# kwea123/nerf_pl

Measured on AMD Instinct MI355X. Metric: rays/sec (64+128 samples), full training step: render_rays fwd + MSE + bwd + grad all-reduce + Adam, higher is better.
Workload: dtype bf16

## Files before the change

### nerf_pl_amd/csrc/mlp_render.hip

```cpp
#include "common.h"
#include "mlp_layout.h"

namespace nerfhip {
using namespace mlp;
typedef nerfhip_render_args RenderArgs;
constexpr int kRenderRays = 4;

template <int PREC, int SV>
int launch_render_variant(const RenderArgs& a, unsigned groups, hipStream_t stream);
template <> int launch_render_variant<NERFHIP_F32, 0>(const RenderArgs&, unsigned, hipStream_t);
template <> int launch_render_variant<NERFHIP_F32, 1>(const RenderArgs&, unsigned, hipStream_t);
template <> int launch_render_variant<NERFHIP_BF16, 0>(const RenderArgs&, unsigned, hipStream_t);
template <> int launch_render_variant<NERFHIP_BF16, 1>(const RenderArgs&, unsigned, hipStream_t);
template <> int launch_render_variant<NERFHIP_BF16, 2>(const RenderArgs&, unsigned, hipStream_t);
template <> int launch_render_variant<NERFHIP_F32, 3>(const RenderArgs&, unsigned, hipStream_t);
template <> int launch_render_variant<NERFHIP_BF16, 3>(const RenderArgs&, unsigned, hipStream_t);

static int render_tail_floats_host(int S_c, int N_i) {
    const int S_f = S_c + N_i;
    const int S4 = (S_c + 3) & ~3, N4 = (N_i + 3) & ~3, F4 = (S_f + 3) & ~3;
    const int fz = N_i > 0 ? 3 * S4 + N4 + ((S_c + 1 + 3) & ~3) + N4 : 0;
    const int coarse = 2 * S4 + fz;
    return coarse > F4 ? coarse : F4;
}

static bool render_shape_ok(int64_t B, int S_c, int N_i, int dtype) {
    if (dtype != NERFHIP_F32 && dtype != NERFHIP_BF16 && dtype != NERFHIP_BF16_F8) return false;
    const int pts = 32 * (dtype == NERFHIP_F32 ? 4 : 8);
    if (B <= 0 || B % kRenderRays != 0 || B / kRenderRays > 0x7fffffff || S_c < 3 || N_i < 0) return false;
    if ((kRenderRays * S_c) % pts != 0 || (N_i > 0 && (kRenderRays * (S_c + N_i)) % pts != 0)) return false;
    if ((int64_t)B * (S_c + N_i) / pts > 0x7fffffff) return false;
    return (size_t)kRenderRays * render_tail_floats_host(S_c, N_i) * sizeof(float) <= (size_t)kSlots * kChunkBytes;
}

static int render_check(const RenderArgs* a, int dtype, bool train) {
    NERFHIP_CHECK_ARG(a != nullptr);
    if (!render_shape_ok(a->B, a->S_c, a->N_i, dtype)) return NERFHIP_E_UNSUPPORTED;
    const bool fine = a->N_i > 0;
    NERFHIP_CHECK_ARG(a->rays && a->packed_coarse && a->z_coarse && a->raw_coarse && a->opacity_coarse);
    NERFHIP_CHECK_ARG(!fine || (a->packed_fine && a->z_fine && a->raw_fine && a->rgb_fine && a->depth_fine && a->opacity_fine));
    NERFHIP_CHECK_ARG(a->perturb <= 0.0f || a->perturb_rand);
    NERFHIP_CHECK_ARG(a->noise_std == 0.0f || (a->noise_coarse && (!fine || a->noise_fine)));
    NERFHIP_CHECK_ARG(a->row_total == NERFHIP_ROW_TOTAL_EXACT || a->row_total == NERFHIP_ROW_TOTAL_ATEN);
    if (train)
        NERFHIP_CHECK_ARG(a->target && a->rgb_coarse && a->depth_coarse && a->g_raw_coarse && a->save_coarse && a->out3 && a->ticket &&
                          (!fine || (a->g_raw_fine && a->save_fine)));
    uintptr_t lines = (uintptr_t)a->z_coarse | (uintptr_t)a->raw_coarse | (uintptr_t)a->z_fine | (uintptr_t)a->raw_fine;
    if (train) lines |= (uintptr_t)a->g_raw_coarse | (uintptr_t)a->g_raw_fine;
    if ((lines & 127) || (((uintptr_t)a->packed_coarse | (uintptr_t)a->packed_fine) & 15)) return NERFHIP_E_ALIGN;
    return 0;
}

}

extern "C" int nerfhip_render_supported(int64_t B, int S_c, int N_i, int dtype) {
    return nerfhip::render_shape_ok(B, S_c, N_i, dtype) ? 1 : 0;
// ... 34 lines not shown
```

### nerf_pl_amd/csrc/mlp_render_kernel.h

```cpp
#pragma once
#include "composite_wave.h"
#include "mlp_fwd_kernel.h"

namespace nerfhip {

constexpr int kRenderRays = 4;

typedef nerfhip_render_args RenderArgs;

__host__ __device__ inline int render_tail_floats(int S_c, int N_i, int S_f) {
    const int S4 = (S_c + 3) & ~3, N4 = (N_i + 3) & ~3, F4 = (S_f + 3) & ~3;
    const int fz = N_i > 0 ? 3 * S4 + N4 + ((S_c + 1 + 3) & ~3) + N4 : 0;
    const int coarse = 2 * S4 + fz;
    return coarse > F4 ? coarse : F4;
}

__device__ __forceinline__ void render_wg_sync() {
    asm volatile("s_waitcnt vmcnt(0) lgkmcnt(0)\n\ts_barrier" ::: "memory");
}

typedef const RenderArgs __attribute__((address_space(4)))* RenderArgsP;
__device__ __forceinline__ RenderArgsP render_args() {
    RenderArgsP p = (RenderArgsP)__builtin_amdgcn_kernarg_segment_ptr();
    asm volatile("" : "+s"(p));
    return p;
}

template <bool TRAIN, int NW, bool TT = false>
__device__ __forceinline__ void render_tail(const bool fine_pass, const bool with_fine_z, float* const tail_lds, const int wave,
                                            const int lane) {
    constexpr int R = kRenderRays;
    const RenderArgsP a = render_args();
    const int S_c = a->S_c, N_i = a->N_i, S_f = S_c + N_i;
    const float noise_std = a->noise_std;
    const float* raw = fine_pass ? a->raw_fine : a->raw_coarse;
    const float* z = fine_pass ? a->z_fine : a->z_coarse;
    const float* noise = noise_std != 0.0f ? (fine_pass ? a->noise_fine : a->noise_coarse) : nullptr;
    const int S = fine_pass ? S_f : S_c;
    float* rgb = fine_pass ? a->rgb_fine : a->rgb_coarse;
    float* depth = fine_pass ? a->depth_fine : a->depth_coarse;
    float* opac = fine_pass ? a->opacity_fine : a->opacity_coarse;
    const float* rays = a->rays;
    const int white_back = a->white_back;
    const int per_ray = render_tail_floats(S_c, N_i, S_f);
    const int S4 = (S_c + 3) & ~3;
    const int64_t ray0 = (int64_t)blockIdx.x * R, B = a->B;
    const int njobs = with_fine_z ? 2 * R : R;
    for (int job = wave; job < njobs; job += NW) {
        const int slot = job < R ? job : job - R;
        const int64_t r = ray0 + slot;
        if (r >= B) continue;
        float* base = tail_lds + (size_t)slot * per_ray;
        if (job < R) {
            if constexpr (TRAIN) {
                composite_train_wave<true>(raw, z, rays, noise, noise_std, white_back, a->target, a->grad_scale, nullptr, rgb, depth, opac,
                                           fine_pass ? a->g_raw_fine : a->g_raw_coarse, r, S, base, nullptr, lane);
            } else if (TT && !fine_pass) {
                composite_fwd_wave<1>(raw, z, rays, noise, noise_std, white_back, nullptr, nullptr, nullptr, opac, r, S, nullptr, lane);
            } else {
                composite_fwd_wave<4>(raw, z, rays, noise, noise_std, white_back, nullptr, rgb, depth, opac, r, S, nullptr, lane);
            }
        } else {
            float* w_s = base + S4;
            composite_weights_wave<(TT ? 1 : 4)>(raw, z, rays, noise, noise_std, r, S, w_s, lane);
            __builtin_amdgcn_wave_barrier();
            const float* u = a->u;
            fine_z_wave(w_s + S4, z + r * S, [&](int j) { return w_s[1 + j]; }, u ? u + r * a->u_stride : nullptr, S, N_i, a->eps,
                        a->z_fine + r * S_f, nullptr, nullptr, nullptr, lane, a->row_total);
        }
    }
}

template <int PREC, int SV>
__global__ __launch_bounds__(PrecTraits<PREC>::NW * 64, PrecTraits<PREC>::WPS)
void mlp_render_kernel(const RenderArgs args_by_value) {
    constexpr bool TRAIN = SV == 1 || SV == 2, TT = SV == 3;
    constexpr int FSV = TT ? 0 : SV;
    constexpr int NW = PrecTraits<PREC>::NW, PTS = 32 * NW, R = kRenderRays;
    __shared__ __attribute__((aligned(1024))) char lds_all[FwdLds<PREC, TRAIN>::kBytes];
    __shared__ float red[2][16];
    __shared__ unsigned last_s;
    const int lane = threadIdx.x & 63;
    const int wave = __builtin_amdgcn_readfirstlane((int)(threadIdx.x >> 6));
    float* const tail_lds = reinterpret_cast<float*>(lds_all + FwdLds<PREC, TRAIN>::kRingOff);
    int nc, nf;
    {
        const RenderArgsP a = render_args();
        const int S_c = a->S_c, N_i = a->N_i;
        nc = R * S_c / PTS;
        nf = N_i > 0 ? R * (S_c + N_i) / PTS : 0;
    }
    const int total = nc + nf;
#pragma clang loop unroll(disable)
    for (int sp = 0; sp < total; ++sp) {
        if (sp > 0) render_wg_sync();
        if (sp == nc) {
            render_tail<TRAIN, NW, TT>(false, true, tail_lds, wave, lane);
            render_wg_sync();
        }
        const RenderArgsP a = render_args();
        const bool fine = sp >= nc;
        const int S = fine ? a->S_c + a->N_i : a->S_c;
        const unsigned blk = fine ? blockIdx.x * (unsigned)nf + (unsigned)(sp - nc) : blockIdx.x * (unsigned)nc + (unsigned)sp;
        const FwdZGen zg{fine ? nullptr : a->perturb_rand, fine ? nullptr : a->z_coarse, fine ? 0 : a->use_disp, fine ? 0.0f : a->perturb,
                          TRAIN ? a->regen_enc : 0};
        uint8_t* save = nullptr;
        if constexpr (TRAIN) save = (uint8_t*)(fine ? a->save_fine : a->save_coarse);
        if (TT && !fine)
            mlp_fwd_body<PREC, MODE_RAYS, true, 0>(lds_all, blk, a->rays, nullptr, a->B * (int64_t)S, (int64_t)S, (const uint8_t*)a->packed_coarse,
                                                   a->raw_coarse, nullptr, zg);
        else
            mlp_fwd_body<PREC, MODE_RAYS, false, FSV>(lds_all, blk, a->rays, fine ? a->z_fine : nullptr, a->B * (int64_t)S, (int64_t)S,
                                                      (const uint8_t*)(fine ? a->packed_fine : a->packed_coarse), fine ? a->raw_fine : a->raw_coarse, save, zg);
    }
    render_wg_sync();
    render_tail<TRAIN, NW, TT>(nf > 0, false, tail_lds, wave, lane);

    if constexpr (TRAIN) {
        const RenderArgsP a = render_args();
        unsigned* const ticket = a->ticket;
        asm volatile("s_waitcnt vmcnt(0)" ::: "memory");
        __syncthreads();
        if (threadIdx.x == 0) {
            const unsigned prev = __hip_atomic_fetch_add(ticket, 1u, __ATOMIC_RELAXED, __HIP_MEMORY_SCOPE_AGENT);
            last_s = (prev == gridDim.x - 1) ? 1u : 0u;
            if (prev == gridDim.x - 1) __hip_atomic_store(ticket, 0u, __ATOMIC_RELAXED, __HIP_MEMORY_SCOPE_AGENT);
        }
        __syncthreads();
        if (!last_s) return;
        __builtin_amdgcn_fence(__ATOMIC_ACQUIRE, "agent");
        const float* img_c = a->rgb_coarse;
        const float* img_f = a->rgb_fine;
        const float* target = a->target;
        float* out3 = a->out3;
        const int64_t n3 = 3 * a->B;
        auto fresh_c = [&](int64_t i) { return __hip_atomic_load(img_c + i, __ATOMIC_RELAXED, __HIP_MEMORY_SCOPE_AGENT); };
        auto fresh_f = [&](int64_t i) { return __hip_atomic_load(img_f + i, __ATOMIC_RELAXED, __HIP_MEMORY_SCOPE_AGENT); };
        constexpr int Q = 1024 / (NW * 64);
        if (nf > 0)
            mse_psnr_block<Q>(fresh_c, fresh_f, true, target, n3, out3, nullptr, nullptr, red);
        else
            mse_psnr_block<Q>(fresh_c, [&](int64_t i) { return 0.0f; }, false, target, n3, out3, nullptr, nullptr, red);
    }
}

template <int PREC, int SV>
int launch_render_variant(const RenderArgs& a, unsigned groups, hipStream_t stream);

}
// ... 1 lines not shown
```

### nerf_pl_amd/csrc/sampling_wave.h

```cpp
#pragma once
#include "sampling_math.h"

namespace nerfhip {

template <typename P>
__device__ __forceinline__ int lower_bound(P a, int n, float v) {
    int lo = 0, hi = n;
    while (lo < hi) {
        const int mid = (lo + hi) >> 1;
        if (a[mid] < v) lo = mid + 1; else hi = mid;
    }
    return lo;
}
template <typename P>
__device__ __forceinline__ int upper_bound(P a, int n, float v) {
    int lo = 0, hi = n;
    while (lo < hi) {
        const int mid = (lo + hi) >> 1;
        if (a[mid] <= v) lo = mid + 1; else hi = mid;
    }
    return lo;
}

constexpr int ROW_TOTAL_EXACT = 0, ROW_TOTAL_ATEN = 1;
// ... 61 lines not shown
        for (int j = lane; j < M; j += 64) part += (double)nh_add(wload(j), eps);
        total = (float)wave_sum(part);
    }
    double carry = 0.0;
    for (int j0 = 0; j0 < M; j0 += 64) {
        const int j = j0 + lane;
        const float pdf = (j < M) ? nh_div(nh_add(wload(j), eps), total) : 0.0f;
        const double incl = wave_incl_sum((double)pdf, lane) + carry;
        if (j < M) cdf_s[j + 1] = (float)incl;
        carry = __shfl(incl, 63, 64);
    }
    if (lane == 0) cdf_s[0] = 0.0f;
    __builtin_amdgcn_wave_barrier();
}

__device__ __forceinline__ float invert_cdf(const float* cdf_s, const float* bins_s, int M, float u, float eps,
                                            int* ind_out = nullptr) {
    const int ind = upper_bound(cdf_s, M + 1, u);
    if (ind_out) *ind_out = ind;
    const int below = max(ind - 1, 0);
    const int above = min(ind, M);
    const float cb = cdf_s[below], ca = cdf_s[above];
    const float bb = bins_s[below], ba = bins_s[above];
    float denom = nh_sub(ca, cb);
    if (denom < eps) denom = 1.0f;
    const float t = nh_div(nh_sub(u, cb), denom);
    return nh_add(bb, nh_mul(t, nh_sub(ba, bb)));
}

__device__ __forceinline__ int fine_z_lds_floats(int S, int N) {
    const int S4 = (S + 3) & ~3, N4 = (N + 3) & ~3;
    return 3 * S4 + N4 + ((S + 1 + 3) & ~3) + N4;
}
template <typename WLoad>
__device__ __forceinline__ void fine_z_wave(float* lds, const float* __restrict__ zrow, WLoad wload, const float* __restrict__ urow,
                                            int S, int N, float eps, float* __restrict__ out, float* __restrict__ znew,
                                            float* __restrict__ cdf_row, int64_t* __restrict__ inds_row, int lane,
                                            int row_total = ROW_TOTAL_EXACT) {
    const int M = S - 2;
    const int S4 = (S + 3) & ~3, N4 = (N + 3) & ~3, H4 = (S + 1 + 3) & ~3;
    float* zc_s = lds;
    float* cdf_s = zc_s + S4;
    float* bins_s = cdf_s + S4;
    float* zn_s = bins_s + S4;
    int* hist_s = reinterpret_cast<int*>(zn_s + N4);
    int* ub_s = hist_s + H4;
    for (int j = lane; j < S; j += 64) zc_s[j] = zrow[j];
    for (int j = lane; j <= S; j += 64) hist_s[j] = 0;
    if (lane < N4 - N) zn_s[N + lane] = __builtin_inff();
    __builtin_amdgcn_wave_barrier();
    for (int j = lane; j < S - 1; j += 64) bins_s[j] = nh_mul(0.5f, nh_add(zc_s[j], zc_s[j + 1]));
    build_cdf_wave(wload, M, eps, cdf_s, lane, row_total);
    if (cdf_row)
        for (int j = lane; j <= M; j += 64) cdf_row[j] = cdf_s[j];
    for (int k = lane; k < N; k += 64) {
        const float uk = urow ? urow[k] : linspace01(k, N);
        int ind;
        const float v = invert_cdf(cdf_s, bins_s, M, uk, eps, &ind);
        if (inds_row) inds_row[k] = (int64_t)ind;
        zn_s[k] = v;
        if (znew) znew[k] = v;
        const int ub = upper_bound(zc_s, S, v);
        ub_s[k] = ub;
        atomicAdd(&hist_s[ub], 1);
    }
    __builtin_amdgcn_wave_barrier();
    int carry = 0;
    for (int i0 = 0; i0 < S; i0 += 64) {
        const int i = i0 + lane;
        int c = (i < S) ? hist_s[i] : 0;
#pragma unroll
        for (int o = 1; o < 64; o <<= 1) {
            const int t = __shfl_up(c, o, 64);
            if (lane >= o) c += t;
        }
        c += carry;
        if (i < S) out[i + c] = zc_s[i];
        carry = __shfl(c, 63, 64);
    }
    bool in_order = true;
    for (int k = lane; k < N; k += 64) in_order = in_order && (k == 0 || zn_s[k - 1] <= zn_s[k]);
    if (__all(in_order)) {
        for (int k = lane; k < N; k += 64) out[ub_s[k] + k] = zn_s[k];
        return;
    }
    const float4* zn4 = reinterpret_cast<const float4*>(zn_s);
    for (int k = lane; k < N; k += 64) {
        const float x = zn_s[k];
        int rank = ub_s[k];
#pragma unroll 4
        for (int q4 = 0; q4 < N4 / 4; ++q4) {
            const float4 y = zn4[q4];
            const int q = q4 * 4;
            rank += (y.x < x || (y.x == x && q + 0 < k)) ? 1 : 0;
            rank += (y.y < x || (y.y == x && q + 1 < k)) ? 1 : 0;
            rank += (y.z < x || (y.z == x && q + 2 < k)) ? 1 : 0;
            rank += (y.w < x || (y.w == x && q + 3 < k)) ? 1 : 0;
        }
        out[rank] = x;
    }
}

}
```

### nerf_pl_amd/csrc/mlp_bwd_chain.hip

```cpp
#include "mlp_device.h"
#include "f8_store.h"
#include "mlp_bwd_chain.h"

namespace nerfhip {

__device__ __forceinline__ float slab_absmax8(const bf16x8& s) {
    float m = 0.0f;
#pragma unroll
    for (int j = 0; j < 8; ++j) m = fmaxf(m, fabsf((float)s[j]));
    return m;
}
__device__ __forceinline__ float slab_absmax8(const f32x8& s) { return 0.0f; }

constexpr int kChainDepthBf16 = 2, kChainDepthF8 = 0;
constexpr int kChainBurst = 2;
template <int PREC> using BwdStream = RingStream<PrecTraits<PREC>::NW, bwd_chunks(PREC), true>;

template <typename Slab>
__device__ __forceinline__ Slab load_slab(__amdgpu_buffer_rsrc_t rsrc, int sec, int lane) {
    Slab s;
    u32x4* dst = reinterpret_cast<u32x4*>(&s);
    const unsigned voff = (unsigned)lane * (unsigned)sizeof(Slab);
    const unsigned soff = (unsigned)(sec * 64 * sizeof(Slab));
#pragma unroll
// ... 203 lines not shown
    st.wave = wave;
    st.pending = 0;
    st.pending_prev = 0;
    st.issue_chunk(0);
    st.issue_chunk(1);
    const unsigned lds_lo = (unsigned)(uintptr_t)ring + (unsigned)lane * 16u;
    unsigned lds_hi = lds_lo + 65536u;
    asm volatile("" : "+v"(lds_hi));
    const unsigned sig_lds = (unsigned)(uintptr_t)ring + (unsigned)(kSlots * kChunkBytes) + (unsigned)((wave * 64 + lane) * (int)sizeof(Slab));

    float v[8];
    Slab zero_slab;
#pragma unroll
    for (int j = 0; j < 8; ++j) v[j] = 0.0f;
    make_slab(zero_slab, v);
    Slab g_rgb, g_sig;
    {
        const float ga[3] = {g.x * o.x * (1.0f - o.x), g.y * o.y * (1.0f - o.y), g.z * o.z * (1.0f - o.z)};
#pragma unroll
        for (int j = 0; j < 8; ++j) v[j] = (h == 0 && j < 3) ? ga[j < 3 ? j : 0] : 0.0f;
        make_slab(g_rgb, v);
#pragma unroll
        for (int j = 0; j < 8; ++j) v[j] = (h == 0 && j == 0) ? g.w : 0.0f;
        make_slab(g_sig, v);
    }
    if constexpr (F8) {
        if constexpr (PREC == NERFHIP_BF16) {
            const int sb_rgb = bf8_block_scale(slab_absmax8(g_rgb)), sb_sig = bf8_block_scale(slab_absmax8(g_sig));
            save_pair_bf8(st.pending, dy_tile, kDyRgb / 2, g_rgb, zero_slab, sb_rgb, lane);
            save_pair_bf8(st.pending, dy_tile, kDySigma / 2, g_sig, zero_slab, sb_sig, lane);
            save_scale_f8(st.pending, dy_tile, f8_dy_scale_off(), f8_dy_section(kDyRgb), sb_rgb, lane);
            save_scale_f8(st.pending, dy_tile, f8_dy_scale_off(), f8_dy_section(kDySigma), sb_sig, lane);
        }
    } else {
        store_slab<PREC>(st.pending, dys, kDyRgb, g_rgb, lane);
        store_slab<PREC>(st.pending, dys, kDyRgb + 1, zero_slab, lane);
        store_slab<PREC>(st.pending, dys, kDySigma, g_sig, lane);
        store_slab<PREC>(st.pending, dys, kDySigma + 1, zero_slab, lane);
    }

    Slab gd[8];
    Slab ga[16], gb[16];
    Slab g_in0[1] = {g_rgb};
    int sb = run_bwd_layer_tm<PREC, 0, 4, 1, true, F8, 0>(st, lds_lo, lds_hi, sig_lds, g_in0, gd, acts, kGateOff, kMaskPieceT, dys, dy_tile, kDyDir,
                                                          f8_dy_section(kDyDir), -1, 127, lane);
    *reinterpret_cast<__attribute__((address_space(3))) Slab*>(sig_lds) = g_sig;
    static_assert(kBwdLayerFold == 1, "layer sequence below");
    sb = run_bwd_layer_tm<PREC, 1, 8, 9, true, F8, 4>(st, lds_lo, lds_hi, sig_lds, gd, gb, acts, kGateOff, mask_piece_h(8), dys, dy_tile, dy_h(8),
                                                      f8_dy_section(dy_h(8)), kDyDir, sb, lane);
    static_assert(bwd_layer_pieces(2, PREC) * 3 % (kChunkPieces * kSlots) == 0, "three looped layers = a whole number of ring turns");
#define NH_BWD(L, IN, OUT, D)                                                                                                \
    sb = run_bwd_layer_tm<PREC, L, 8, 16, true, F8, 8>(st, lds_lo, lds_hi, sig_lds, reinterpret_cast<const Slab(&)[16]>(IN), OUT, acts, kGateOff, \
                                                       mask_piece_h(9 - L) - (D), dys, dy_tile, dy_h(9 - L) + 16 * (D),              \
                                                       f8_dy_section(dy_h(9 - L)) + (D), dy_h(10 - L) + 16 * (D), sb, lane);
    if constexpr (PREC != NERFHIP_BF16) {
        NH_BWD(2, gb, ga, 0) NH_BWD(3, ga, gb, 0) NH_BWD(4, gb, ga, 0) NH_BWD(5, ga, gb, 0) NH_BWD(6, gb, ga, 0) NH_BWD(7, ga, gb, 0)
    } else {
        const uint8_t* const gsrc0 = st.gsrc;
        int n_pass;
        asm volatile("s_mov_b32 %0, 2" : "=s"(n_pass));
#pragma clang loop unroll(disable)
        for (int pass = 0; pass < n_pass; ++pass) {
            st.pending = 0;
            st.pending_prev = 0;
            const int d = 3 * pass;
            NH_BWD(2, gb, ga, d) NH_BWD(3, ga, gb, d) NH_BWD(4, gb, ga, d)
// ... 49 lines not shown
```

### nerf_pl_amd/csrc/mlp_bwd_dw.hip

```cpp
#include "mlp_device.h"
#include "mlp_bwd_dw.h"

namespace nerfhip {

#if NERFHIP_DW_PROBE
__device__ unsigned g_dw_probe[1024 * 8 * 8];
#endif

constexpr int kDwRingKiB = 160, kDwMaxDepth = 12;
constexpr int kDwFragRing = 5, kDwFragRing2D = 4;

template <int PREC> struct DwTraits;
template <> struct DwTraits<NERFHIP_BF16> {
    static constexpr int SPP = 1;
    static constexpr int RING_BYTES = kDwRingKiB * 1024;
    static constexpr int DEPTH = 0, STAGE_BYTES = 0;
};
template <> struct DwTraits<NERFHIP_F32> {
    static constexpr int SPP = 2;
    static constexpr int DEPTH = 2;
    static constexpr int MAXP = 72;
    static constexpr int STAGE_BYTES = MAXP * kPieceBytes;
    static constexpr int RING_BYTES = DEPTH * STAGE_BYTES;
};
// ... 76 lines not shown
    const int64_t my_tiles = (t_first >= ntiles) ? 0 : ((ntiles - t_first < per) ? ntiles - t_first : per);
    const unsigned lds_base = (unsigned)(uintptr_t)ring;

    const int dma_off_even = (PREC == NERFHIP_BF16) ? ((lane & 1) * 32 + (lane >> 1)) * 16 : lane * 16;
    const int dma_off_odd = (PREC == NERFHIP_BF16) ? ((lane & 1) * 32 + ((lane ^ 8) >> 1)) * 16 : lane * 16;

    f32x16 acc[kDwMaxXTiles];
#pragma unroll
    for (int x = 0; x < kDwMaxXTiles; ++x)
#pragma unroll
        for (int r = 0; r < 16; ++r) acc[x][r] = 0.0f;
    float dbacc = 0.0f;
    [[maybe_unused]] float dbacc2 = 0.0f;

    const int grp = lane >> 4, c = lane & 15;
    const int tr_off = (grp & 1) * SLAB_BYTES + (2 * (8 * (grp >> 1) + (c >> 2)) + ((c & 3) & 1)) * 16 + ((c & 3) >> 1) * 8;
    const int tr_s0 = (grp & 1) ? 128 : 0, tr_s1 = 128 - tr_s0;
    [[maybe_unused]] auto load_frag = [&](const char* pb, int q) { return load_frag_tr16(pb, tr_off, tr_s0, tr_s1, q); };
    const int m32 = lane & 31, kk = lane >> 5;
    const int f32_off = (m32 >> 4) * SLAB_BYTES + (slab_nat_h(m32 & 15) * 32) * 32 + slab_nat_j(m32 & 15) * 4;
#if NERFHIP_DW_PROBE
    unsigned pr_wait = 0, pr_bar = 0, pr_issue = 0, pr_comp = 0, pr_depth = 0;
    const uint64_t pr_t00 = __builtin_amdgcn_s_memrealtime();
#endif

    auto run = [&](auto nxt_c, auto nsl_c, auto regen_c) {
        constexpr int NXT = decltype(nxt_c)::value, NSL = decltype(nsl_c)::value;
        constexpr bool REGEN = decltype(regen_c)::value;
        static_assert(!REGEN || (PREC == NERFHIP_BF16 && (NXT == 2 || NXT == 9 || NXT == 10)), "classes with an encoding section");
        constexpr int ENC = REGEN ? (NXT == 9 ? kDirSlabs : kXyzSlabs) : 0;
        constexpr int DYS = NXT == 9 ? 8 : 16;
        constexpr bool FOLD = NXT == 9 && NSL == kDwFoldStageSlabs;
        constexpr bool SPLIT2D = (PREC == NERFHIP_BF16) && (NXT == 8 || NXT == 10) && (NSL - 2 * NXT >= 16);
        constexpr int NP = NSL * SPP;
        constexpr int NPD = NP - ENC;
        constexpr int LPWD = (NPD + 7) / 8;
        constexpr int LPW = LPWD + (REGEN ? 1 : 0);
        constexpr int STAGE = (PREC == NERFHIP_BF16) ? NP * kPieceBytes : DwTraits<PREC>::STAGE_BYTES;
        constexpr int ZSLOT = 256;
        constexpr int D0 = dw_depth<PREC>(NP);
        constexpr int D = (REGEN && D0 * (STAGE + ZSLOT) > RING_BYTES) ? D0 - 1 : D0;
        static_assert(D >= 2 && D * (STAGE + (REGEN ? ZSLOT : 0)) <= RING_BYTES, "ring stages of this job class");
        static_assert((D - 2) * LPW <= 63, "counted vmcnt");
#if NERFHIP_DW_PROBE
        pr_depth = D;
#endif
        int s_issue = 0, s_use = 0;
        const uint8_t* abase = nullptr;
        const uint8_t* dbase = nullptr;
        unsigned slot = 0;
        auto stage_tile = [&](int64_t it) {
            int64_t T = t_first + (it < my_tiles ? it : my_tiles - 1);
            if (T >= ntiles) T = ntiles - 1;
            return T;
        };
        const float* zsrc = nullptr;
        unsigned zslot = 0;
        int z_issue = 0, g_slot = 0;
        const unsigned lds_z = lds_base + (unsigned)(D * STAGE);
        auto next_z = [&](int64_t st) {
            zsrc = enc_z + stage_tile(st) * 32 + (lane & 31);
            zslot = (unsigned)__builtin_amdgcn_readfirstlane((int)(lds_z + (unsigned)(z_issue * ZSLOT)));
            z_issue = (z_issue + 1 == D) ? 0 : z_issue + 1;
        };
        auto next_stage = [&](int64_t it) {
            const int64_t T = stage_tile(it);
            abase = acts_base + tile_block_off(T, act_tile_bytes(PREC), IL);
            dbase = dys_base + tile_block_off(T, kDySlabs * 64 * (16 * SPP), IL);
            slot = lds_base + (unsigned)(s_issue * STAGE);
// ... 1 lines not shown
            if constexpr (REGEN) next_z(it + 1);
        };
        float ray_next[6] = {0.f, 0.f, 0.f, 0.f, 0.f, 0.f};
        auto load_ray = [&](int64_t st) {
            if (wave < ENC) {
                const unsigned r = (unsigned)__builtin_amdgcn_readfirstlane((int)((unsigned)stage_tile(st) / (unsigned)enc_tpr));
                typedef const float __attribute__((address_space(4))) * ConstF;
                const ConstF rp = (ConstF)(uintptr_t)(enc_rays + (size_t)r * 8);
#pragma unroll
                for (int c = 0; c < 6; ++c) ray_next[c] = rp[c];
            }
        };
        auto gen_stage = [&](int64_t st) {
            if (wave < ENC) {
                const int n = lane & 31, h = lane >> 5;
                bf16x8 e;
                if constexpr (NXT == 9) {
                    const float dv[3] = {ray_next[3], ray_next[4], ray_next[5]};
                    e = dw_encode_slab<4, kDirSlabs>(dv, h, wave);
                } else {
                    const float zv = *reinterpret_cast<const float*>(ring + D * STAGE + g_slot * ZSLOT + n * 4);
                    float xv[3];
#pragma unroll
                    for (int c = 0; c < 3; ++c) xv[c] = nh_add(ray_next[c], nh_mul(ray_next[3 + c], zv));
                    e = dw_encode_slab<10, kXyzSlabs>(xv, h, wave);
                }
                const int unit = (2 * n + h) ^ ((wave & 1) ? 8 : 0);
                *reinterpret_cast<bf16x8*>(ring + g_slot * STAGE + (DYS + wave) * SLAB_BYTES + unit * 16) = e;
            }
            g_slot = (g_slot + 1 == D) ? 0 : g_slot + 1;
            load_ray(st + 1);
        };
        constexpr int REM = NPD % 8;
        constexpr bool SHARE_LAST = (PREC == NERFHIP_BF16) && (REM == 4 || REM == 2);
        const int share_piece = NPD - REM + (SHARE_LAST ? (wave * REM) / 8 : 0);
        const unsigned long long share_mask = REM == 4 ? (0xffffffffull << (32 * (wave & 1))) : (0xffffull << (16 * (wave & 3)));
        auto issue_piece = [&](int i) {
            if constexpr (REGEN) {
                if (i == LPW - 1) {
                    glds4(zsrc, zslot);
                    return;
                }
            }
            int pi = wave + 8 * i;
            const bool shared = SHARE_LAST && i == LPWD - 1;
            if (shared) pi = share_piece;
            if (pi >= NPD) pi = NPD - 1;
            if (REGEN && pi >= DYS) pi += ENC;
            const int sl = pi / SPP, sub = pi % SPP;
            const uint8_t* src;
            if (FOLD && sl >= kDwFoldSigmaSlab) src = dbase + (size_t)(kDySigma + sl - kDwFoldSigmaSlab) * 64 * (16 * SPP) * IL;
            else if (sl < jb.dy_slabs) src = dbase + (size_t)(jb.dy_off + sl) * 64 * (16 * SPP) * IL;
            else if (sl < jb.dy_slabs + jb.x1_slabs) src = abase + (size_t)(jb.x1_off + sl - jb.dy_slabs) * 64 * (16 * SPP) * IL;
            else src = abase + (size_t)(jb.x2_off + sl - jb.dy_slabs - jb.x1_slabs) * 64 * (16 * SPP) * IL;
            const uint8_t* g = src + (size_t)sub * kPieceBytes + ((sl & 1) ? dma_off_odd : dma_off_even);
            const unsigned dst = (unsigned)__builtin_amdgcn_readfirstlane((int)(slot + (unsigned)(pi * kPieceBytes)));
            if (shared) glds16_nt_masked(g, dst, share_mask);
            else glds16_nt(g, dst);
        };
        auto issue_stage = [&](int64_t it) {
            next_stage(it);
#pragma unroll
            for (int i = 0; i < LPW; ++i) issue_piece(i);
        };
        constexpr bool SPREAD = (PREC == NERFHIP_BF16);
        constexpr int DMA_STEP = (2 * NXT) / LPW > 0 ? (2 * NXT) / LPW : 1;
        if constexpr (REGEN) {
            next_z(0);
            glds4(zsrc, zslot);
            load_ray(0);
        }
#pragma unroll
        for (int s = 0; s < D - 1; ++s) issue_stage(s);
        if constexpr (REGEN) {
            wait_vm<(D - 1) * LPW>();
            gen_stage(0);
        }
        for (int64_t it = 0; it < my_tiles; ++it) {
#if NERFHIP_DW_PROBE
            const unsigned t0 = shader_cycles();
            wait_vm<(PREC == NERFHIP_BF16) ? (D - 2) * LPW : 0>();
            const unsigned t1 = shader_cycles();
            asm volatile("s_barrier" ::: "memory");
            const unsigned t2 = shader_cycles();
            pr_wait += (t1 - t0) & 0xffffffffu;
            pr_bar += (t2 - t1) & 0xffffffffu;
#else
            wait_vm_barrier<(PREC == NERFHIP_BF16) ? (D - 2) * LPW : 0>();
#endif
            if (SPREAD && (SPLIT2D || wave < n_ot)) next_stage(it + D - 1);
            else issue_stage(it + D - 1);
#if NERFHIP_DW_PROBE
            const unsigned t3 = shader_cycles();
            pr_issue += (t3 - t2) & 0xffffffffu;
#endif
            const char* st_base = ring + s_use * STAGE;
            s_use = (s_use + 1 == D) ? 0 : s_use + 1;
            if constexpr (SPLIT2D) {
                constexpr int XW = NXT / 2, NF = 2 * XW, RD = kDwFragRing2D;
// ... 201 lines not shown
```

### nerf_pl_amd/models/mlp_autograd.py

```python
import torch

from .. import ops


def _param_grads(model, out, acts, dtype, g_out, packed_bwd, workspace=None):
    gw, gb, flat = ops.mlp_bwd(g_out, out, packed_bwd, acts, dtype, workspace=workspace)
    model._flat_grad = flat
    hook = getattr(model, "_grad_ready_hook", None)
    if hook is not None:
        hook(model, flat)
    need = [p.requires_grad for p in model.flat_params()]
    return [g if nd else None for g, nd in zip(gw + gb, need)]


def _needs_grad(model):
    return torch.is_grad_enabled() and any(p.requires_grad for p in model.parameters())


class _MLPRays(torch.autograd.Function):

    @staticmethod
    def forward(ctx, model, rays, z, *params):
        dtype = model.mlp_dtype
        acts = ops.alloc_acts(z.numel(), dtype, z.device)
# ... 2 lines not shown
        ctx.model, ctx.dtype, ctx.acts, ctx.packed_bwd = model, dtype, acts, packed_bwd
        ctx.serial = model._packed_serial
        ctx.save_for_backward(out)
        return out

    @staticmethod
    def backward(ctx, g_out):
        (out,) = ctx.saved_tensors
        ctx.model.check_pack_serial(ctx.serial)
        grads = _param_grads(ctx.model, out, ctx.acts, ctx.dtype, g_out, ctx.packed_bwd)
        ctx.acts = ctx.packed_bwd = None
        return (None, None, None) + tuple(grads)


class _MLPEmbedded(torch.autograd.Function):

    @staticmethod
    def forward(ctx, model, x, *params):
        dtype = model.mlp_dtype
        if dtype == "bf16_f8" and ctx.needs_input_grad[1]:
            dtype = "bf16"
        acts = ops.alloc_acts(x.shape[0], dtype, x.device)
        packed, packed_bwd = model.packed_weights_train(dtype)
        out = ops.mlp_fwd_embedded(x, packed, False, dtype, save=acts)
        ctx.model, ctx.dtype, ctx.acts, ctx.packed_bwd = model, dtype, acts, packed_bwd
        ctx.serial = model._packed_serial
        ctx.save_for_backward(out)
        return out

    @staticmethod
    def backward(ctx, g_out):
        (out,) = ctx.saved_tensors
        ctx.model.check_pack_serial(ctx.serial)
        ws = {} if ctx.needs_input_grad[1] else None
        grads = _param_grads(ctx.model, out, ctx.acts, ctx.dtype, g_out, ctx.packed_bwd, workspace=ws)
        ctx.acts = ctx.packed_bwd = None
        gx = None
        if ctx.needs_input_grad[1]:
            m = ctx.model
            gx = ops.mlp_dx_embedded(ws["dys"], out.shape[0], m.xyz_encoding_1[0].weight, m.xyz_encoding_5[0].weight,
                                     m.dir_encoding[0].weight, ctx.dtype)
        return (None, gx) + tuple(grads)


def mlp_rays(model, rays, z, sigma_only):
    if _needs_grad(model):
        out = _MLPRays.apply(model, rays, z, *model.flat_params())
        return out[..., 3] if sigma_only else out
    return ops.mlp_fwd_rays(rays, z, model.packed_weights(), sigma_only, model.mlp_dtype)


def mlp_embedded(model, x, sigma_only):
    lead = x.shape[:-1]
    x2 = x.reshape(-1, x.shape[-1]).float()
    if _needs_grad(model) or (torch.is_grad_enabled() and x2.requires_grad):
        if sigma_only:
            if x2.shape[1] != model.in_channels_xyz:
                raise ValueError("NeRF.forward expects %d input channels, got %d" % (model.in_channels_xyz, x2.shape[1]))
            x2 = torch.cat([x2, x2.new_zeros(x2.shape[0], model.in_channels_dir)], 1)
            out = _MLPEmbedded.apply(model, x2, *model.flat_params())[:, 3:4]
        else:
            out = _MLPEmbedded.apply(model, x2, *model.flat_params())
    else:
        out = ops.mlp_fwd_embedded(x2, model.packed_weights(), sigma_only, model.mlp_dtype)
    return out.reshape(*lead, out.shape[-1])
```

### nerf_pl_amd/ops.py

```python
import ctypes
import os

import torch

from . import _lib
from ._lib import BF16, BF16_F8, F32, NerfHipError, check, device_guard, ptr, require_gpu, stream_ptr

_DTYPES = {"fp32": F32, "f32": F32, "float32": F32, torch.float32: F32, F32: F32,
           "bf16": BF16, "bfloat16": BF16, torch.bfloat16: BF16, "bf16_f8": BF16_F8}


def mlp_dtype_code(d):
    if isinstance(d, bool) or d not in _DTYPES:
        raise ValueError("mlp dtype must be 'fp32', 'bf16' or 'bf16_f8', got %r" % (d,))
    return _DTYPES[d]


def _c(t):
    return t if t.is_contiguous() else t.contiguous()


def _check_draw(op, name, t, numel):
    if t is not None and (t.numel() != numel or t.dtype != torch.float32):
        raise ValueError("%s: %s must hold %d fp32 draws, got %s %s" % (op, name, numel, tuple(t.shape), t.dtype))
# ... 531 lines not shown
    return bufs


FLAT_GRAD_FLOATS = sum(s[0] * s[1] + s[0] for s in PARAM_SHAPES)


def flat_grad_views(n_points, device, shapes=PARAM_SHAPES, out=None):
    sizes = [s[0] * s[1] for s in shapes] + [s[0] for s in shapes]
    if out is not None:
        flat = out
        if n_points == 0:
            flat.zero_()
    else:
        flat = (torch.zeros if n_points == 0 else torch.empty)(sum(sizes), device=device, dtype=torch.float32)
    views, off = [], 0
    for sz in sizes:
        views.append(flat[off:off + sz])
        off += sz
    return [v.view(s) for v, s in zip(views[:12], shapes)], views[12:], flat


@device_guard
def mlp_bwd(g_out, out, packed_bwd, acts, dtype, shapes=PARAM_SHAPES, phases=7, workspace=None):
    require_gpu(g_out, out)
    code = mlp_dtype_code(dtype)
    g_out = _c(g_out.float()).reshape(-1, 4)
    out = _c(out).reshape(-1, 4)
    n = out.shape[0]
    dev = out.device
    lib = _lib.load()
    if workspace is not None and "dys" in workspace:
        dys, ws = workspace["dys"], workspace["ws"]
    else:
        dys = torch.empty(int(lib.nerfhip_mlp_dy_bytes(n, code)), device=dev, dtype=torch.uint8)
        ws = torch.empty(int(lib.nerfhip_mlp_dw_workspace_bytes(n, code)), device=dev, dtype=torch.uint8)
        if workspace is not None:
            workspace["dys"], workspace["ws"] = dys, ws
    gw, gb, flat = flat_grad_views(n, dev, shapes)
    gwp = (ctypes.c_void_p * 12)(*[t.data_ptr() for t in gw])
    gbp = (ctypes.c_void_p * 12)(*[t.data_ptr() for t in gb])
    check(lib.nerfhip_mlp_bwd_phases(ptr(g_out), ptr(out), n, ptr(packed_bwd), ptr(acts), ptr(dys), ptr(ws), gwp, gbp, 0, code,
                                     int(phases), stream_ptr()), "nerfhip_mlp_bwd")
    return gw, gb, flat


@device_guard
def mlp_dx_embedded(dys, n, w_xyz1, w_xyz5, w_dir, dtype):
    code = mlp_dtype_code(dtype)
    if code == BF16_F8:
        raise NotImplementedError("nerfhip_mlp_dx_embedded reads bf16 / fp32 dY slabs ('bf16_f8' keeps dY only as e5m2: NeRF.forward "
                                  "saves in bf16 for calls whose input requires grad, models/mlp_autograd.py)")
    require_gpu(w_xyz1, w_xyz5, w_dir)
    gx = torch.empty(n, 90, device=dys.device, dtype=torch.float32)
    check(_lib.load().nerfhip_mlp_dx_embedded(ptr(dys), n, ptr(_c(w_xyz1.detach())), ptr(_c(w_xyz5.detach())), ptr(_c(w_dir.detach())),
                                              ptr(gx), 90, code, stream_ptr()), "nerfhip_mlp_dx_embedded")
    return gx


def pack_tables(models, dtype):
    if not 1 <= len(models) <= 4:
        raise ValueError("pack_models_train packs 1..4 models")
    tabs, bufs = [], []
    for m in models:
        if not m.is_default_arch():
            raise NotImplementedError(DEFAULT_ARCH_ONLY)
        wp, bp, dev = m._pack_args()
        tabs.append((wp, bp))
# ... 20 lines not shown
    return bufs


def mlp_bwd_multi(entries, dtype, adam=None, phases=7, workspace=None, g_scale=None):
    code = mlp_dtype_code(dtype)
    lib = _lib.load()
    M = len(entries)
    dev = entries[0][1].device
    gs, outs, ns, dys, grads = [], [], [], [], []
    enc, keep_enc = None, []
    for m, e in enumerate(entries):
        g_out, out = e[0], e[1]
        if len(e) > 4 and e[4] is not None:
            if enc is None:
                enc = _lib.EncSource()
            rays_e, z_e = _c(e[4]), _c(e[5])
            require_gpu(rays_e, z_e)
            if rays_e.dtype != torch.float32 or z_e.dtype != torch.float32 or z_e.dim() != 2 or rays_e.shape[0] != z_e.shape[0]:
                raise ValueError("mlp_bwd_multi: (rays (B,8), z (B,S)) fp32 expected")
            enc.rays[m], enc.z[m], enc.S[m] = rays_e.data_ptr(), z_e.data_ptr(), int(z_e.shape[1])
            keep_enc.append((rays_e, z_e))
        require_gpu(g_out, out)
        g_out = _c(g_out.float()).reshape(-1, 4)
        out = _c(out).reshape(-1, 4)
        gs.append(g_out)
        outs.append(out)
        ns.append(out.shape[0])
    with torch.cuda.device(dev):
        n_arr = (ctypes.c_int64 * M)(*ns)
        key = ("multi", tuple(ns), code)
        if workspace is not None and key in workspace:
            dys, ws = workspace[key]
        else:
            dys = [torch.empty(int(lib.nerfhip_mlp_dy_bytes(n, code)), device=dev, dtype=torch.uint8) for n in ns]
            ws = torch.empty(int(lib.nerfhip_mlp_dw_workspace_bytes_multi(n_arr, M, code)), device=dev, dtype=torch.uint8)
            if workspace is not None:
                workspace[key] = (dys, ws)
        joint = torch.empty(M * FLAT_GRAD_FLOATS, device=dev, dtype=torch.float32)
        for m, n in enumerate(ns):
            grads.append(flat_grad_views(n, dev, out=joint[m * FLAT_GRAD_FLOATS:(m + 1) * FLAT_GRAD_FLOATS]))
        vp = ctypes.c_void_p
        G = (vp * M)(*[t.data_ptr() for t in gs])
        O = (vp * M)(*[t.data_ptr() for t in outs])
        PB = (vp * M)(*[e[2].data_ptr() for e in entries])
        AC = (vp * M)(*[e[3].data_ptr() for e in entries])
        DY = (vp * M)(*[t.data_ptr() for t in dys])
        GW = (vp * (12 * M))(*[t.data_ptr() for g in grads for t in g[0]])
        GB = (vp * (12 * M))(*[t.data_ptr() for g in grads for t in g[1]])
        if adam is not None:
            for m in range(M):
                adam.grad_flat[m] = grads[m][2].data_ptr()
        if g_scale is not None:
            require_gpu(g_scale)
        check(lib.nerfhip_mlp_bwd_multi_rays(M, G, O, n_arr, PB, AC, DY, ptr(ws), GW, GB, 0, code, int(phases), ptr(g_scale),
                                             ctypes.addressof(adam) if adam is not None else None,
                                             ctypes.addressof(enc) if enc is not None else None, stream_ptr()), "nerfhip_mlp_bwd_multi_rays")
    return grads


ACT_NONE, ACT_RELU, ACT_SIGMOID = 0, 1, 2


def _rows(t):
    if t.dim() != 2:
        raise ValueError("expected a (n, channels) tensor")
    if t.stride(1) != 1 or t.stride(0) < t.shape[1]:
        t = t.contiguous()
# ... 459 lines not shown
```

Before: 1.076 million.

## Split fine-z sampling across two waves per ray and run final composites concurrently

```diff
diff --git a/nerf_pl_amd/csrc/mlp_render.hip b/nerf_pl_amd/csrc/mlp_render.hip
--- a/nerf_pl_amd/csrc/mlp_render.hip
+++ b/nerf_pl_amd/csrc/mlp_render.hip
@@ -20,8 +20,8 @@
     const int S_f = S_c + N_i;
     const int S4 = (S_c + 3) & ~3, N4 = (N_i + 3) & ~3, F4 = (S_f + 3) & ~3;
     const int fz = N_i > 0 ? 3 * S4 + N4 + ((S_c + 1 + 3) & ~3) + N4 : 0;
-    const int coarse = 2 * S4 + fz;
-    return coarse > F4 ? coarse : F4;
+    const int boundary = 2 * S4 + fz, final_tail = F4 + (N_i > 0 ? S4 : 0);
+    return boundary > final_tail ? boundary : final_tail;
 }
 
 static bool render_shape_ok(int64_t B, int S_c, int N_i, int dtype) {
diff --git a/nerf_pl_amd/csrc/mlp_render_kernel.h b/nerf_pl_amd/csrc/mlp_render_kernel.h
--- a/nerf_pl_amd/csrc/mlp_render_kernel.h
+++ b/nerf_pl_amd/csrc/mlp_render_kernel.h
@@ -11,8 +11,8 @@
 __host__ __device__ inline int render_tail_floats(int S_c, int N_i, int S_f) {
     const int S4 = (S_c + 3) & ~3, N4 = (N_i + 3) & ~3, F4 = (S_f + 3) & ~3;
     const int fz = N_i > 0 ? 3 * S4 + N4 + ((S_c + 1 + 3) & ~3) + N4 : 0;
-    const int coarse = 2 * S4 + fz;
-    return coarse > F4 ? coarse : F4;
+    const int boundary = 2 * S4 + fz, final_tail = F4 + (N_i > 0 ? S4 : 0);
+    return boundary > final_tail ? boundary : final_tail;
 }
 
 __device__ __forceinline__ void render_wg_sync() {
@@ -26,47 +26,74 @@
     return p;
 }
 
+template <int NW, bool TT>
+__device__ __forceinline__ void render_fine_z_tail(float* const tail_lds, int wave, int lane) {
+    constexpr int R = kRenderRays, PARTS = NW >= 2 * R ? 2 : 1;
+    asm volatile("" : "+s"(wave), "+v"(lane));
+    const RenderArgsP a = render_args();
+    const int S_c = a->S_c, N_i = a->N_i, S_f = S_c + N_i;
+    const int S4 = (S_c + 3) & ~3;
+    const int slot = wave % R, part = wave / R;
+    const int64_t r = (int64_t)blockIdx.x * R + slot;
+    const bool mine = part < PARTS && r < a->B;
+    float* const w_s = tail_lds + (size_t)slot * render_tail_floats(S_c, N_i, S_f) + S4;
+    const FineZLds L = fine_z_lds(w_s + S4, S_c, N_i);
+    const float* z = a->z_coarse;
+    if (mine) {
+        if (part == PARTS - 1) fine_z_prep(L, z + r * S_c, S_c, N_i, lane);
+        if (part == 0) {
+            const float noise_std = a->noise_std;
+            composite_weights_wave<(TT ? 1 : 4)>(a->raw_coarse, z, a->rays, noise_std != 0.0f ? a->noise_coarse : nullptr, noise_std, r, S_c, w_s,
+                                                 lane);
+            __builtin_amdgcn_wave_barrier();
+            build_cdf_wave([&](int j) { return w_s[1 + j]; }, S_c - 2, a->eps, L.cdf_s, lane, a->row_total);
+        }
+    }
+    __syncthreads();
+    if (mine) {
+        const float* u = a->u;
+        fine_z_draws(L, u ? u + r * a->u_stride : nullptr, S_c, N_i, a->eps, part * 64 + lane, PARTS * 64, nullptr, nullptr);
+    }
+    __syncthreads();
+    if (mine) {
+        float* out = a->z_fine + r * S_f;
+        if (part == 0) fine_z_merge_coarse(L, S_c, out, lane);
+        fine_z_merge_new(L, N_i, out, part * 64 + lane, PARTS * 64, lane);
+    }
+}
+
 template <bool TRAIN, int NW, bool TT = false>
-__device__ __forceinline__ void render_tail(const bool fine_pass, const bool with_fine_z, float* const tail_lds, const int wave,
-                                            const int lane) {
+__device__ __forceinline__ void render_composite_tail(const bool with_fine, float* const tail_lds, const int wave, const int lane) {
     constexpr int R = kRenderRays;
     const RenderArgsP a = render_args();
     const int S_c = a->S_c, N_i = a->N_i, S_f = S_c + N_i;
     const float noise_std = a->noise_std;
-    const float* raw = fine_pass ? a->raw_fine : a->raw_coarse;
-    const float* z = fine_pass ? a->z_fine : a->z_coarse;
-    const float* noise = noise_std != 0.0f ? (fine_pass ? a->noise_fine : a->noise_coarse) : nullptr;
-    const int S = fine_pass ? S_f : S_c;
-    float* rgb = fine_pass ? a->rgb_fine : a->rgb_coarse;
-    float* depth = fine_pass ? a->depth_fine : a->depth_coarse;
-    float* opac = fine_pass ? a->opacity_fine : a->opacity_coarse;
     const float* rays = a->rays;
     const int white_back = a->white_back;
     const int per_ray = render_tail_floats(S_c, N_i, S_f);
-    const int S4 = (S_c + 3) & ~3;
+    const int F4 = (S_f + 3) & ~3;
     const int64_t ray0 = (int64_t)blockIdx.x * R, B = a->B;
-    const int njobs = with_fine_z ? 2 * R : R;
+    const int njobs = with_fine ? 2 * R : R;
     for (int job = wave; job < njobs; job += NW) {
+        const bool fine_pass = with_fine && job < R;
         const int slot = job < R ? job : job - R;
         const int64_t r = ray0 + slot;
         if (r >= B) continue;
-        float* base = tail_lds + (size_t)slot * per_ray;
-        if (job < R) {
-            if constexpr (TRAIN) {
-                composite_train_wave<true>(raw, z, rays, noise, noise_std, white_back, a->target, a->grad_scale, nullptr, rgb, depth, opac,
-                                           fine_pass ? a->g_raw_fine : a->g_raw_coarse, r, S, base, nullptr, lane);
-            } else if (TT && !fine_pass) {
-                composite_fwd_wave<1>(raw, z, rays, noise, noise_std, white_back, nullptr, nullptr, nullptr, opac, r, S, nullptr, lane);
-            } else {
-                composite_fwd_wave<4>(raw, z, rays, noise, noise_std, white_back, nullptr, rgb, depth, opac, r, S, nullptr, lane);
-            }
+        const float* raw = fine_pass ? a->raw_fine : a->raw_coarse;
+        const float* z = fine_pass ? a->z_fine : a->z_coarse;
+        const float* noise = noise_std != 0.0f ? (fine_pass ? a->noise_fine : a->noise_coarse) : nullptr;
+        const int S = fine_pass ? S_f : S_c;
+        float* rgb = fine_pass ? a->rgb_fine : a->rgb_coarse;
+        float* depth = fine_pass ? a->depth_fine : a->depth_coarse;
+        float* opac = fine_pass ? a->opacity_fine : a->opacity_coarse;
+        float* T_s = tail_lds + (size_t)slot * per_ray + (job < R ? 0 : F4);
+        if constexpr (TRAIN) {
+            composite_train_wave<true>(raw, z, rays, noise, noise_std, white_back, a->target, a->grad_scale, nullptr, rgb, depth, opac,
+                                       fine_pass ? a->g_raw_fine : a->g_raw_coarse, r, S, T_s, nullptr, lane);
+        } else if (TT && !fine_pass) {
+            composite_fwd_wave<1>(raw, z, rays, noise, noise_std, white_back, nullptr, nullptr, nullptr, opac, r, S, nullptr, lane);
         } else {
-            float* w_s = base + S4;
-            composite_weights_wave<(TT ? 1 : 4)>(raw, z, rays, noise, noise_std, r, S, w_s, lane);
-            __builtin_amdgcn_wave_barrier();
-            const float* u = a->u;
-            fine_z_wave(w_s + S4, z + r * S, [&](int j) { return w_s[1 + j]; }, u ? u + r * a->u_stride : nullptr, S, N_i, a->eps,
-                        a->z_fine + r * S_f, nullptr, nullptr, nullptr, lane, a->row_total);
+            composite_fwd_wave<4>(raw, z, rays, noise, noise_std, white_back, nullptr, rgb, depth, opac, r, S, nullptr, lane);
         }
     }
 }
@@ -95,7 +122,7 @@
     for (int sp = 0; sp < total; ++sp) {
         if (sp > 0) render_wg_sync();
         if (sp == nc) {
-            render_tail<TRAIN, NW, TT>(false, true, tail_lds, wave, lane);
+            render_fine_z_tail<NW, TT>(tail_lds, wave, lane);
             render_wg_sync();
         }
         const RenderArgsP a = render_args();
@@ -114,7 +141,7 @@
                                                       (const uint8_t*)(fine ? a->packed_fine : a->packed_coarse), fine ? a->raw_fine : a->raw_coarse, save, zg);
     }
     render_wg_sync();
-    render_tail<TRAIN, NW, TT>(nf > 0, false, tail_lds, wave, lane);
+    render_composite_tail<TRAIN, NW, TT>(nf > 0, tail_lds, wave, lane);
 
     if constexpr (TRAIN) {
         const RenderArgsP a = render_args();
diff --git a/nerf_pl_amd/csrc/sampling_wave.h b/nerf_pl_amd/csrc/sampling_wave.h
--- a/nerf_pl_amd/csrc/sampling_wave.h
+++ b/nerf_pl_amd/csrc/sampling_wave.h
@@ -117,62 +117,75 @@
     const int S4 = (S + 3) & ~3, N4 = (N + 3) & ~3;
     return 3 * S4 + N4 + ((S + 1 + 3) & ~3) + N4;
 }
-template <typename WLoad>
-__device__ __forceinline__ void fine_z_wave(float* lds, const float* __restrict__ zrow, WLoad wload, const float* __restrict__ urow,
-                                            int S, int N, float eps, float* __restrict__ out, float* __restrict__ znew,
-                                            float* __restrict__ cdf_row, int64_t* __restrict__ inds_row, int lane,
-                                            int row_total = ROW_TOTAL_EXACT) {
+struct FineZLds {
+    float* zc_s;
+    float* cdf_s;
+    float* bins_s;
+    float* zn_s;
+    int* hist_s;
+    int* ub_s;
+};
+__device__ __forceinline__ FineZLds fine_z_lds(float* lds, int S, int N) {
+    const int S4 = (S + 3) & ~3, N4 = (N + 3) & ~3, H4 = (S + 1 + 3) & ~3;
+    FineZLds L;
+    L.zc_s = lds;
+    L.cdf_s = L.zc_s + S4;
+    L.bins_s = L.cdf_s + S4;
+    L.zn_s = L.bins_s + S4;
+    L.hist_s = reinterpret_cast<int*>(L.zn_s + N4);
+    L.ub_s = L.hist_s + H4;
+    return L;
+}
+__device__ __forceinline__ void fine_z_prep(const FineZLds& L, const float* __restrict__ zrow, int S, int N, int lane) {
+    const int N4 = (N + 3) & ~3;
+    for (int j = lane; j < S; j += 64) L.zc_s[j] = zrow[j];
+    for (int j = lane; j <= S; j += 64) L.hist_s[j] = 0;
+    if (lane < N4 - N) L.zn_s[N + lane] = __builtin_inff();
+    __builtin_amdgcn_wave_barrier();
+    for (int j = lane; j < S - 1; j += 64) L.bins_s[j] = nh_mul(0.5f, nh_add(L.zc_s[j], L.zc_s[j + 1]));
+}
+__device__ __forceinline__ void fine_z_draws(const FineZLds& L, const float* __restrict__ urow, int S, int N, float eps, int k0, int kstep,
+                                             float* __restrict__ znew, int64_t* __restrict__ inds_row) {
     const int M = S - 2;
-    const int S4 = (S + 3) & ~3, N4 = (N + 3) & ~3, H4 = (S + 1 + 3) & ~3;
-    float* zc_s = lds;
-    float* cdf_s = zc_s + S4;
-    float* bins_s = cdf_s + S4;
-    float* zn_s = bins_s + S4;
-    int* hist_s = reinterpret_cast<int*>(zn_s + N4);
-    int* ub_s = hist_s + H4;
-    for (int j = lane; j < S; j += 64) zc_s[j] = zrow[j];
-    for (int j = lane; j <= S; j += 64) hist_s[j] = 0;
-    if (lane < N4 - N) zn_s[N + lane] = __builtin_inff();
-    __builtin_amdgcn_wave_barrier();
-    for (int j = lane; j < S - 1; j += 64) bins_s[j] = nh_mul(0.5f, nh_add(zc_s[j], zc_s[j + 1]));
-    build_cdf_wave(wload, M, eps, cdf_s, lane, row_total);
-    if (cdf_row)
-        for (int j = lane; j <= M; j += 64) cdf_row[j] = cdf_s[j];
-    for (int k = lane; k < N; k += 64) {
+    for (int k = k0; k < N; k += kstep) {
         const float uk = urow ? urow[k] : linspace01(k, N);
         int ind;
-        const float v = invert_cdf(cdf_s, bins_s, M, uk, eps, &ind);
+        const float v = invert_cdf(L.cdf_s, L.bins_s, M, uk, eps, &ind);
         if (inds_row) inds_row[k] = (int64_t)ind;
-        zn_s[k] = v;
+        L.zn_s[k] = v;
         if (znew) znew[k] = v;
-        const int ub = upper_bound(zc_s, S, v);
-        ub_s[k] = ub;
-        atomicAdd(&hist_s[ub], 1);
-    }
-    __builtin_amdgcn_wave_barrier();
+        const int ub = upper_bound(L.zc_s, S, v);
+        L.ub_s[k] = ub;
+        atomicAdd(&L.hist_s[ub], 1);
+    }
+}
+__device__ __forceinline__ void fine_z_merge_coarse(const FineZLds& L, int S, float* __restrict__ out, int lane) {
     int carry = 0;
     for (int i0 = 0; i0 < S; i0 += 64) {
         const int i = i0 + lane;
-        int c = (i < S) ? hist_s[i] : 0;
+        int c = (i < S) ? L.hist_s[i] : 0;
 #pragma unroll
         for (int o = 1; o < 64; o <<= 1) {
             const int t = __shfl_up(c, o, 64);
             if (lane >= o) c += t;
         }
         c += carry;
-        if (i < S) out[i + c] = zc_s[i];
+        if (i < S) out[i + c] = L.zc_s[i];
         carry = __shfl(c, 63, 64);
     }
+}
+__device__ __forceinline__ void fine_z_merge_new(const FineZLds& L, int N, float* __restrict__ out, int k0, int kstep, int lane) {
+    const int N4 = (N + 3) & ~3;
     bool in_order = true;
-    for (int k = lane; k < N; k += 64) in_order = in_order && (k == 0 || zn_s[k - 1] <= zn_s[k]);
+    for (int k = lane; k < N; k += 64) in_order = in_order && (k == 0 || L.zn_s[k - 1] <= L.zn_s[k]);
     if (__all(in_order)) {
-        for (int k = lane; k < N; k += 64) out[ub_s[k] + k] = zn_s[k];
+        for (int k = k0; k < N; k += kstep) out[L.ub_s[k] + k] = L.zn_s[k];
         return;
     }
-    const float4* zn4 = reinterpret_cast<const float4*>(zn_s);
-    for (int k = lane; k < N; k += 64) {
-        const float x = zn_s[k];
-        int rank = ub_s[k];
+    const float4* zn4 = reinterpret_cast<const float4*>(L.zn_s);
+    for (int k = k0; k < N; k += kstep) {
+        const float x = L.zn_s[k];
+        int rank = L.ub_s[k];
 #pragma unroll 4
         for (int q4 = 0; q4 < N4 / 4; ++q4) {
             const float4 y = zn4[q4];
@@ -186,4 +199,21 @@
     }
 }
 
-}
+template <typename WLoad>
+__device__ __forceinline__ void fine_z_wave(float* lds, const float* __restrict__ zrow, WLoad wload, const float* __restrict__ urow,
+                                            int S, int N, float eps, float* __restrict__ out, float* __restrict__ znew,
+                                            float* __restrict__ cdf_row, int64_t* __restrict__ inds_row, int lane,
+                                            int row_total = ROW_TOTAL_EXACT) {
+    const int M = S - 2;
+    const FineZLds L = fine_z_lds(lds, S, N);
+    fine_z_prep(L, zrow, S, N, lane);
+    build_cdf_wave(wload, M, eps, L.cdf_s, lane, row_total);
+    if (cdf_row)
+        for (int j = lane; j <= M; j += 64) cdf_row[j] = L.cdf_s[j];
+    fine_z_draws(L, urow, S, N, eps, lane, 64, znew, inds_row);
+    __builtin_amdgcn_wave_barrier();
+    fine_z_merge_coarse(L, S, out, lane);
+    fine_z_merge_new(L, N, out, lane, 64, lane);
+}
+
+}
```

New measurement: 1.080 million (median of 6 runs). No clear change (+0.4%).

## Store only the live half of the bf16 output-gradient seed slabs and zero-fill the rest in LDS

Applied to the files above, without the earlier changes.

```diff
diff --git a/nerf_pl_amd/csrc/mlp_bwd_chain.hip b/nerf_pl_amd/csrc/mlp_bwd_chain.hip
--- a/nerf_pl_amd/csrc/mlp_bwd_chain.hip
+++ b/nerf_pl_amd/csrc/mlp_bwd_chain.hip
@@ -259,6 +259,13 @@
             save_scale_f8(st.pending, dy_tile, f8_dy_scale_off(), f8_dy_section(kDyRgb), sb_rgb, lane);
             save_scale_f8(st.pending, dy_tile, f8_dy_scale_off(), f8_dy_section(kDySigma), sb_sig, lane);
         }
+    } else if constexpr (PREC == NERFHIP_BF16) {
+        __amdgpu_buffer_rsrc_t seed_rgb = __builtin_amdgcn_make_buffer_rsrc(dy_tile + (size_t)kDyRgb * 64 * sizeof(Slab) * IL, 0,
+                                                                             32 * (int)sizeof(Slab), 0x00020000);
+        __amdgpu_buffer_rsrc_t seed_sig = __builtin_amdgcn_make_buffer_rsrc(dy_tile + (size_t)kDySigma * 64 * sizeof(Slab) * IL, 0,
+                                                                             32 * (int)sizeof(Slab), 0x00020000);
+        store_slab_b128(st.pending, seed_rgb, g_rgb, (unsigned)lane * (unsigned)sizeof(Slab));
+        store_slab_b128(st.pending, seed_sig, g_sig, (unsigned)lane * (unsigned)sizeof(Slab));
     } else {
         store_slab<PREC>(st.pending, dys, kDyRgb, g_rgb, lane);
         store_slab<PREC>(st.pending, dys, kDyRgb + 1, zero_slab, lane);
diff --git a/nerf_pl_amd/csrc/mlp_bwd_dw.hip b/nerf_pl_amd/csrc/mlp_bwd_dw.hip
--- a/nerf_pl_amd/csrc/mlp_bwd_dw.hip
+++ b/nerf_pl_amd/csrc/mlp_bwd_dw.hip
@@ -132,9 +132,12 @@
         constexpr int DYS = NXT == 9 ? 8 : 16;
         constexpr bool FOLD = NXT == 9 && NSL == kDwFoldStageSlabs;
         constexpr bool SPLIT2D = (PREC == NERFHIP_BF16) && (NXT == 8 || NXT == 10) && (NSL - 2 * NXT >= 16);
+        constexpr bool SEED = (PREC == NERFHIP_BF16) && (FOLD || (NXT == 4 && NSL == 10));
+        constexpr int HP = FOLD ? kDwFoldSigmaSlab : 0;
+        static_assert(!SEED || (HP % 2 == 0 && (HP == 0 || HP + 2 == NSL)), "a seed pair leads or ends the stage image");
         constexpr int NP = NSL * SPP;
-        constexpr int NPD = NP - ENC;
-        constexpr int LPWD = (NPD + 7) / 8;
+        constexpr int NPD = NP - ENC - (SEED ? 2 : 0);
+        constexpr int LPWD = SEED ? NPD / 8 + 1 : (NPD + 7) / 8;
         constexpr int LPW = LPWD + (REGEN ? 1 : 0);
         constexpr int STAGE = (PREC == NERFHIP_BF16) ? NP * kPieceBytes : DwTraits<PREC>::STAGE_BYTES;
         constexpr int ZSLOT = 256;
@@ -202,9 +205,13 @@
             load_ray(st + 1);
         };
         constexpr int REM = NPD % 8;
-        constexpr bool SHARE_LAST = (PREC == NERFHIP_BF16) && (REM == 4 || REM == 2);
-        const int share_piece = NPD - REM + (SHARE_LAST ? (wave * REM) / 8 : 0);
-        const unsigned long long share_mask = REM == 4 ? (0xffffffffull << (32 * (wave & 1))) : (0xffffull << (16 * (wave & 3)));
+        static_assert(!SEED || REM == 0 || REM == 2, "the last round of a seed class");
+        constexpr bool SHARE_LAST = (PREC == NERFHIP_BF16) && (SEED || REM == 4 || REM == 2);
+        const bool seed_half = SEED && wave >= 2 * REM;
+        const int share_piece = NPD - REM + (SEED ? (seed_half ? 0 : wave >> 1) : (SHARE_LAST ? (wave * REM) / 8 : 0));
+        const unsigned long long share_mask =
+            SEED ? (REM == 2 ? (seed_half ? (0x5555ull << (16 * (wave & 3))) : (0xffffffffull << (32 * (wave & 1)))) : (0x55ull << (8 * wave)))
+                 : (REM == 4 ? (0xffffffffull << (32 * (wave & 1))) : (0xffffull << (16 * (wave & 3))));
         auto issue_piece = [&](int i) {
             if constexpr (REGEN) {
                 if (i == LPW - 1) {
@@ -216,7 +223,9 @@
             const bool shared = SHARE_LAST && i == LPWD - 1;
             if (shared) pi = share_piece;
             if (pi >= NPD) pi = NPD - 1;
+            if (SEED && HP == 0) pi += 2;
             if (REGEN && pi >= DYS) pi += ENC;
+            if (SEED && shared && seed_half) pi = HP;
             const int sl = pi / SPP, sub = pi % SPP;
             const uint8_t* src;
             if (FOLD && sl >= kDwFoldSigmaSlab) src = dbase + (size_t)(kDySigma + sl - kDwFoldSigmaSlab) * 64 * (16 * SPP) * IL;
@@ -235,6 +244,13 @@
         };
         constexpr bool SPREAD = (PREC == NERFHIP_BF16);
         constexpr int DMA_STEP = (2 * NXT) / LPW > 0 ? (2 * NXT) / LPW : 1;
+        if constexpr (SEED) {
+            for (int u = (int)threadIdx.x; u < D * 96; u += 512) {
+                const int d = u / 96, r = u % 96;
+                const int off = d * STAGE + (r < 32 ? HP * kPieceBytes + (2 * r + 1) * 16 : (HP + 1) * kPieceBytes + (r - 32) * 16);
+                *reinterpret_cast<u32x4*>(ring + off) = u32x4{0u, 0u, 0u, 0u};
+            }
+        }
         if constexpr (REGEN) {
             next_z(0);
             glds4(zsrc, zslot);
diff --git a/nerf_pl_amd/models/mlp_autograd.py b/nerf_pl_amd/models/mlp_autograd.py
--- a/nerf_pl_amd/models/mlp_autograd.py
+++ b/nerf_pl_amd/models/mlp_autograd.py
@@ -58,7 +58,7 @@
     def backward(ctx, g_out):
         (out,) = ctx.saved_tensors
         ctx.model.check_pack_serial(ctx.serial)
-        ws = {} if ctx.needs_input_grad[1] else None
+        ws = {"kernels_only": True} if ctx.needs_input_grad[1] else None
         grads = _param_grads(ctx.model, out, ctx.acts, ctx.dtype, g_out, ctx.packed_bwd, workspace=ws)
         ctx.acts = ctx.packed_bwd = None
         gx = None
diff --git a/nerf_pl_amd/ops.py b/nerf_pl_amd/ops.py
--- a/nerf_pl_amd/ops.py
+++ b/nerf_pl_amd/ops.py
@@ -587,7 +587,8 @@
     if workspace is not None and "dys" in workspace:
         dys, ws = workspace["dys"], workspace["ws"]
     else:
-        dys = torch.empty(int(lib.nerfhip_mlp_dy_bytes(n, code)), device=dev, dtype=torch.uint8)
+        keep = workspace is not None and not workspace.get("kernels_only")
+        dys = (torch.zeros if keep else torch.empty)(int(lib.nerfhip_mlp_dy_bytes(n, code)), device=dev, dtype=torch.uint8)
         ws = torch.empty(int(lib.nerfhip_mlp_dw_workspace_bytes(n, code)), device=dev, dtype=torch.uint8)
         if workspace is not None:
             workspace["dys"], workspace["ws"] = dys, ws
@@ -674,7 +675,8 @@
         if workspace is not None and key in workspace:
             dys, ws = workspace[key]
         else:
-            dys = [torch.empty(int(lib.nerfhip_mlp_dy_bytes(n, code)), device=dev, dtype=torch.uint8) for n in ns]
+            dys = [(torch.zeros if workspace is not None else torch.empty)(int(lib.nerfhip_mlp_dy_bytes(n, code)), device=dev, dtype=torch.uint8)
+                   for n in ns]
             ws = torch.empty(int(lib.nerfhip_mlp_dw_workspace_bytes_multi(n_arr, M, code)), device=dev, dtype=torch.uint8)
             if workspace is not None:
                 workspace[key] = (dys, ws)
```

New measurement: 1.098 million before, 1.111 million after (median of 6 runs). 1.2% higher.
